# ShadowLive/ExtIO_sddc

Hardware: AMD Instinct MI355X
Metric: input MSamples/s at decim=2 + achieved % HBM roofline, 1 GPU; IQ max-rel-err (higher is better)
Workload: dtype f32 (int16 in, complex64 out)

## Files before the change

### extio_sddc_amd/csrc/ddc_fs.hip

```cpp
#include <hip/hip_runtime.h>

#include <type_traits>

#include "ddc_frame_common.hpp"
#include "ddc_queue.hpp"
#include "ddc_stamps.hpp"
#include "ddc_fs_perm.h"

namespace sddc {
namespace {

#ifdef SDDC_STAMPS
__device__ unsigned g_fs_stamps[2048 * 4 * kStampWords];
#endif

__device__ __forceinline__ float dpp_partner(float v)
{
    return __int_as_float(__builtin_amdgcn_mov_dpp(__float_as_int(v), 0xB1, 0xF, 0xF, true));
}

__device__ __forceinline__ void split_v2(float2 &za, float2 &vb, float2 zb, float ra, float rb)
{
    asm("s_nop 1\n\t"
        "v_fmac_f32_dpp %2, %1, %7 quad_perm:[1,0,3,2] row_mask:0xf bank_mask:0xf\n\t"
// ... 43 lines not shown
}

constexpr int kQWave = 3;
constexpr int kFsPqAhead = 1;
__device__ __forceinline__ int fs_row_slot(int t) { return 272 * (t >> 4) + (t >= 128) + 34 * ((t & 15) >> 1) + (t & 1); }
__device__ __forceinline__ int fs_pair_row(int t) { return 2 * (t >> 5) + (t & 1); }
__device__ __forceinline__ int fs_pair_col(int t) { return (t >> 1) & 15; }
__device__ __forceinline__ int fs_pair_slot(int t) { return t + 2 * (t >> 5); }
constexpr int kFsLds = 4352;
constexpr int kFsTw = NT + 1;

enum { kSchedStatic = 0, kSchedQueue = 1, kSchedSteal = 2 };
template <int SCHED> struct SchedOf { using T = StealSchedule; };
template <> struct SchedOf<kSchedStatic> { using T = StaticSchedule; };
template <> struct SchedOf<kSchedQueue> { using T = FrameSchedule<1>; };

template <int ZR>
__device__ __forceinline__ constexpr bool zrow(int k) { return zr_row<ZR>(k); }

template <int SCHED, int ZR, bool RAND, bool LSB, bool NCO, bool CS16>
__global__ __launch_bounds__(NT, 4) void r2iq_fs_kernel(
    const int *__restrict__ in32, void *__restrict__ out, int nframes, const float2 *__restrict__ tw_p1,
    const float2 *__restrict__ rec_f, const float4 *__restrict__ pqf, const float2 *__restrict__ fsl, int tunebin,
    OutArgs oa, NcoArgs nco, unsigned *__restrict__ wq, int ns, unsigned slotw, int xmap, int minrem, int pub)
{
    __shared__ __attribute__((aligned(16))) float2 lds[kFsLds];
    __shared__ __attribute__((aligned(16))) float2 twl[15 * 16];
    __shared__ __attribute__((aligned(16))) float2 wtab[2 * kFsTw];
    __shared__ int s_next;
    static_assert(sizeof(float2) * (kFsLds + 15 * 16 + 2 * kFsTw) + sizeof(int) <= 163840 / 4,
                  "four workgroups per CU");

    const int tid = (int)threadIdx.x;
    const int w = xmap ? (int)(blockIdx.x & 7u) * (int)(gridDim.x >> 3) + (int)(blockIdx.x >> 3) : (int)blockIdx.x;
    constexpr int QLANE = 64 * kQWave;
    const bool qw = __builtin_amdgcn_readfirstlane(tid >> 6) == kQWave;
    typename SchedOf<SCHED>::T fsch;
    int x[16];
    {
        const int G = (int)gridDim.x, a0 = slot_split(ns, G, w, slotw);
        const int f0s = a0 < slot_split(ns, G, w + 1, slotw) ? a0 : -1;
        if (f0s >= 0) load_frame(in32, f0s / FRAMES, f0s % FRAMES, x);
        if (qw) {
            int f0[1];
            if constexpr (SCHED == kSchedSteal) fsch.init(wq, nframes, ns, w, G, slotw, f0, minrem, pub);
            else fsch.init(wq, nframes, ns, w, G, slotw, f0);
            if (tid == QLANE) s_next = f0[0];
        }
        for (int i = tid; i < 15 * 16; i += NT) twl[i] = tw_p1[i];
        wtab[tid + (tid >= 128)] = rec_f[tid];
        wtab[kFsTw + tid + (tid >= 128)] = rec_f[NT + tid];
        __syncthreads();
        const int f = s_next;
        if (f >= 0 && f0s < 0) load_frame(in32, f / FRAMES, f % FRAMES, x);
    }
    int f = s_next;
    int blk = f / FRAMES, k = f - blk * FRAMES;
    const int col_ = kFsPerm[tid];
    const int qt = (tunebin >> 2) & 3;
    const bool w0 = __builtin_amdgcn_readfirstlane(tid >> 6) == 0;
    float cr[16];
    {
        const __amdgpu_buffer_rsrc_t rr = buf_rsrc(reinterpret_cast<const float *>(pqf) + 2 * HALF);
#pragma unroll
        for (int k = 0; k < 16; k++)
            if (!zrow<ZR>(k)) cr[k] = __uint_as_float(__builtin_amdgcn_raw_buffer_load_b32(rr, 4u * tid, 4u * NT * k, 0));
    }
    constexpr int AZR = ZR > 0 ? ZR : -ZR;
    constexpr int CPP = SCHED == kSchedStatic && !NCO && !CS16 && AZR >= 3 ? (AZR >= 4 && AZR <= 7 ? AZR + 1 : AZR) : 0;
    float2 cp[16];
    if constexpr (CPP > 0) {
        const __amdgpu_buffer_rsrc_t rq = buf_rsrc(pqf);
#pragma unroll
        for (int k = 0; k < 16; k++)
            if (!zrow<ZR>(k) && (k < CPP || 15 - k < CPP))
                cp[k] = buf_load8(rq, 16u * tid, 4096u * (k < 8 ? k : 15 - k) + (k < 8 ? 0u : 8u));
    }
    constexpr bool GREG = SCHED == kSchedStatic;
    float2 cg0, cg1, cg4;
    if constexpr (GREG) {
        const __amdgpu_buffer_rsrc_t rfs = buf_rsrc(fsl);
        const unsigned t8 = 8u * (unsigned)tid;
        cg0 = buf_load8(rfs, t8, 0);
        cg1 = buf_load8(rfs, t8, 8u * NT);
        cg4 = buf_load8(rfs, t8, 16u * NT);
    }
    int pA = -1, fend = -1;
    {
        const int G = (int)gridDim.x, a = slot_split(ns, G, w, slotw), b = slot_split(ns, G, w + 1, slotw);
        if constexpr (SCHED == kSchedStatic) {
            pA = b + 2;
            fend = b;
        } else if constexpr (SCHED == kSchedSteal) {
            const int len = b - a, two = len < 2 ? len : 2;
            pA = minrem <= 0 ? b + 2 : a + (pub > 0 && len - pub > two ? len - pub : two);
            fend = minrem <= 0 ? b : pA;
        }
    }
    ST_INIT();

    auto frame = [&](auto phase) __attribute__((always_inline)) {
        constexpr bool PB = decltype(phase)::value;
        if constexpr (PB && SCHED != kSchedSteal)
            if (qw) fsch.peek();
        int z = 0;
        asm volatile("" : "+s"(z));
        const int t = tid + z;
        const int c = col_ + z;
        const int oblk = blk * 8 * HALF;
        const int kc = k;
        float2 v[16];
        {
// ... 191 lines not shown
            const int fb = oblk + emit_base<HALF>(kc);
            switch (qt) {
            case 0: emit_frame_q<0, LSB, NCO, CS16>(out, fb, kc, t, u, oa, nco); break;
            case 1: emit_frame_q<1, LSB, NCO, CS16>(out, fb, kc, t, u, oa, nco); break;
            case 2: emit_frame_q<2, LSB, NCO, CS16>(out, fb, kc, t, u, oa, nco); break;
            default: emit_frame_q<3, LSB, NCO, CS16>(out, fb, kc, t, u, oa, nco); break;
            }
        }
        if constexpr (SCHED == kSchedSteal) {
            if constexpr (PB)
                if (qw) fsch.take_late();
        }
        ST_FRAME_END();
        f = fn;
    };
    if constexpr (SCHED != kSchedQueue)
        while (f >= 0 && f + 2 < pA) frame(std::false_type{});
    if constexpr (SCHED != kSchedStatic) {
        if constexpr (SCHED == kSchedSteal)
            if (qw) fsch.enter(f);
        while (f >= 0) frame(std::true_type{});
    }
    ST_WRITE(g_fs_stamps, w, tid);
    if constexpr (SCHED == kSchedQueue)
        if (tid == QLANE) fs_queue_done(wq, (unsigned)gridDim.x);
}

__global__ void build_fs_tables_kernel(const float2 *__restrict__ hsel0, const float2 *__restrict__ post8192,
                                       const float2 *__restrict__ tw4096, int tunebin, float4 *__restrict__ pqf,
                                       float2 *__restrict__ fsl)
{
    const int i = (int)(blockIdx.x * blockDim.x + threadIdx.x);
    if (i >= HALF) return;
    const int l = i & (NT - 1), kk = i >> 8;
    const int b = kFsPerm[l] + NT * kk;
    const bool band = (b >= tunebin && b - tunebin < HALF / 2) || (b < tunebin && tunebin - b <= HALF / 2);
    float3 c = make_float3(0.f, 0.f, 0.f);
    if (band) {
        const int m = (b - tunebin) & (HALF - 1);
        const double hr = hsel0[m].x, hi = hsel0[m].y;
        const double wr = post8192[b].x, wi = post8192[b].y;
        const double pr = 1.0 + wi, pi = -wr, qr = 1.0 - wi, qi = wr;
        if (b == HALF / 2) {
            c.x = (float)(hr * qr - hi * qi);
            c.y = (float)(hr * qi + hi * qr);
        } else {
// ... 6 lines not shown
    reinterpret_cast<float *>(pqf)[2 * HALF + i] = c.z;
    if (i < NT) {
        fsl[i] = tw4096[(tunebin * i) & (HALF - 1)];
        fsl[NT + i] = tw4096[((tunebin - 1) * i) & (HALF - 1)];
        fsl[2 * NT + i] = tw4096[((tunebin - 4) * i) & (HALF - 1)];
    }
}

template <int SCHED, int ZR, bool RAND, bool LSB, bool NCO, bool CS16>
hipError_t launch_fs_s(const KernelTables &t, const int16_t *d_in, int nblk, void *d_out, const float4 *pqf,
                       const float2 *fsl, int tunebin, const OutArgs &oa, const NcoArgs &nco, unsigned *wq,
                       const FsSched &fs, int device, hipStream_t s)
{
    auto kern = r2iq_fs_kernel<SCHED, ZR, RAND, LSB, NCO, CS16>;
    const int static_pct = SCHED == kSchedQueue ? fs.static_pct : 100, fpw = fs.fpw;
    int occ = 0, cus = 0;
    hipError_t e = launch_geometry(t.lc, reinterpret_cast<const void *>(kern), NT, device, &occ, &cus);
    if (e != hipSuccess) return e;
    const int nframes = nblk * FRAMES;
    int grid = cus * occ;
    if (grid > nframes) grid = nframes;
    int ns = frame_schedule_static(nframes, static_pct);
    unsigned slotw = occ == 4 && grid == cus * occ ? (fs.slotw ? fs.slotw : kFsSlotWeights) : 0u;
    int xmap = 0;
    if (fpw > 0) {
        grid = (nframes + fpw - 1) / fpw;
        ns = nframes;
        slotw = 0u;
        xmap = (grid & 7) == 0 && grid * fpw == nframes;
    }
    int minrem = fs.minrem;
    if (SCHED == kSchedSteal && (grid > kFsStealMax || 2LL * nframes / grid + 1 > kStealMaxRange)) minrem = 0;
    hipLaunchKernelGGL(kern, dim3((unsigned)grid), dim3(NT), 0, s, reinterpret_cast<const int *>(d_in), d_out, nframes,
                       t.tw_p1, t.rec_f, pqf, fsl, tunebin, oa, nco, wq, ns, slotw, xmap, minrem, fs.pub);
    return hipGetLastError();
}

int fs_zero_rows(int tunebin)
{
    const int top = 16 - (tunebin + 2048 + 255) / 256, bot = tunebin > 2048 ? (tunebin - 2048) / 256 : 0;
    const int z = top > 0 ? top : bot > 0 ? -bot : 0;
    return z > 8 ? 8 : z < -8 ? -8 : z == 1 || z == -1 ? 0 : z;
}

template <int ZR, bool RAND, bool LSB, bool NCO, bool CS16>
hipError_t launch_fs_z(const KernelTables &t, const int16_t *d_in, int nblk, void *d_out, const float4 *pqf,
                       const float2 *fsl, int tunebin, const OutArgs &oa, const NcoArgs &nco, unsigned *wq,
                       const FsSched &fs, int device, hipStream_t s)
{
    if (fs.sched == kSchedStatic)
        return launch_fs_s<kSchedStatic, ZR, RAND, LSB, NCO, CS16>(t, d_in, nblk, d_out, pqf, fsl, tunebin, oa, nco, wq, fs, device, s);
    if constexpr (!RAND && !LSB && !NCO && !CS16 && ZR % 4 == 0) {
        if (fs.sched == kSchedSteal)
            return launch_fs_s<kSchedSteal, ZR, false, false, false, false>(t, d_in, nblk, d_out, pqf, fsl, tunebin, oa, nco, wq, fs, device, s);
        if (fs.sched == kSchedQueue)
            return launch_fs_s<kSchedQueue, ZR, false, false, false, false>(t, d_in, nblk, d_out, pqf, fsl, tunebin, oa, nco, wq, fs, device, s);
    }
// ... 80 lines not shown
```

### extio_sddc_amd/csrc/ddc_kernels.h

```cpp
#pragma once

#include <hip/hip_runtime_api.h>
#include <hip/hip_vector_types.h>
#include <stddef.h>
#include <stdint.h>

namespace sddc {

struct LaunchCache {
    static constexpr int kSlots = 256;
    int cus = 0;
    int n = 0;
    const void *fn[kSlots] = {};
    int occ[kSlots] = {};
};

inline hipError_t launch_geometry(LaunchCache *lc, const void *fn, int threads, int device, int *occ, int *cus)
{
    if (lc) {
        for (int i = 0; i < lc->n; i++)
            if (lc->fn[i] == fn) {
                *occ = lc->occ[i];
                *cus = lc->cus;
                return hipSuccess;
            }
    }
    int nb = 0, c = 0;
    hipError_t e = hipOccupancyMaxActiveBlocksPerMultiprocessor(&nb, fn, threads, 0);
// ... 28 lines not shown
                                    const float2 *nco_trig, int slot_weights, int device, hipStream_t s);
constexpr unsigned slot_weights4(unsigned a, unsigned b, unsigned c, unsigned e) { return a | (b << 8) | (c << 16) | (e << 24); }
constexpr unsigned kSlotWeights[7] = {slot_weights4(31, 26, 18, 13), slot_weights4(31, 26, 18, 13), slot_weights4(31, 26, 18, 13),
                                      slot_weights4(29, 25, 20, 15), slot_weights4(29, 25, 20, 15),
                                      slot_weights4(29, 25, 20, 15), slot_weights4(29, 25, 20, 15)};
constexpr int kSlotWeighting = 1;
hipError_t launch_build_split_filter(const KernelTables &t, int d, int tunebin, float4 *pq, hipStream_t s);

bool fs_path(int d, int tunebin);
hipError_t launch_build_fs_tables(const KernelTables &t, int tunebin, float4 *pqf, float2 *fsl, hipStream_t s);
constexpr int kFsQueueLineWords = 16 * 9;
constexpr int kFsStealMax = 2048;
constexpr int kFsQueueWords = kFsQueueLineWords + 2 * kFsStealMax;
constexpr int kFsStaticPct = 100;
constexpr unsigned kFsSlotWeights = slot_weights4(31, 26, 18, 13);
struct FsSched {
    int sched = 0;
    int static_pct = kFsStaticPct;
    int fpw = 0;
    int minrem = 1;
    int pub = 0;
    int zr = 1;
    unsigned slotw = 0u;
};
hipError_t launch_frames_fs(const KernelTables &t, const int16_t *d_in, int nblk, void *d_out, const float4 *pqf,
                            const float2 *fsl, int tunebin, int lsb, int rand, int cs16, float cs16_scale,
                            const float2 *nco_starts, const float2 *nco_trig, unsigned *wq, const FsSched &fs,
                            int device, hipStream_t s);

struct ChNco {
    const float2 *starts = nullptr;
    const float2 *trig = nullptr;
    const float *fc = nullptr;
    int nb = 0;
};
hipError_t launch_channel_nco_chain(float2 *d_state, const float2 *d_trig, float2 *d_starts, int nch, int nb,
                                    hipStream_t s);

hipError_t launch_channels_v2(const KernelTables &t, int d, const int16_t *d_in, int nblk, const int *d_tunebins,
                              int nch, void *d_out, size_t stride, int lsb, int rand, int cs16, float cs16_scale,
                              const int2 *d_windows, float2 *d_scratch, int scratch_rows, int device,
                              hipStream_t s, const ChNco *nco = nullptr);
hipError_t launch_channels_p(const KernelTables &t, int d, const int16_t *d_in, int nblk, const int *d_tunebins,
                             int nch, void *d_out, size_t stride, int lsb, int rand, int cs16, float cs16_scale,
                             float2 *d_scratch, int scratch_rows, int device, hipStream_t s,
                             const ChNco *nco = nullptr);
// ... 8 lines not shown
```

### extio_sddc_amd/csrc/ddc_queue.hpp

```cpp
#pragma once

#include <hip/hip_runtime.h>

#include "ddc_device_io.hpp"

namespace sddc {
namespace {

constexpr int FS_SHARDS = 8;
static_assert(kFsQueueLineWords == 16 * (FS_SHARDS + 1), "queue slot: one 64-B line per shard counter + the done count");
constexpr unsigned FS_OOB = 0x80000000u;

__device__ __forceinline__ int slot_split(int ns, int G, int v, unsigned slotw)
{
    if (slotw == 0u || (G & 3)) return (int)(((long long)ns * v) / G);
    const int Q = G >> 2, q = v / Q, i = v - q * Q;
    long long sw = 0, tot = 0;
#pragma unroll
    for (int k = 0; k < 4; k++) {
        const int wk = (int)((slotw >> (8 * k)) & 0xffu);
        tot += (long long)Q * wk;
        if (k < q) sw += (long long)Q * wk;
        else if (k == q) sw += (long long)i * wk;
    }
    return (int)(((long long)ns * sw) / tot);
}

struct FsQueue {
    __amdgpu_buffer_rsrc_t rq;
    int base, nd;
    int sh0;
    int shn;
    int lo, cnt;
    int tk;
    int pv;

    __device__ __forceinline__ int shard_lo(int s) const { return base + ((nd * s) >> 3); }
    __device__ __forceinline__ void init(unsigned *wq, int base_, int nd_, int home)
    {
        rq = __builtin_amdgcn_make_buffer_rsrc(wq, (short)0, 4 * kFsQueueLineWords, 0x00020000);
        base = base_;
        nd = nd_;
        sh0 = home;
        set_shard(0);
    }
    __device__ __forceinline__ void set_shard(int sh)
    {
        shn = sh;
// ... 51 lines not shown
        }
        rem = b - a - LA;
        nxt = a + LA;
        if (rem <= 0) q.take();
    }
    __device__ __forceinline__ void peek()
    {
        if (rem <= 0) q.peek();
    }
    __device__ __forceinline__ int next()
    {
        const int fn = rem > 0 ? nxt++ : q.resolve();
        rem--;
        return fn;
    }
    __device__ __forceinline__ void take()
    {
        if (rem <= 0) q.take();
    }
};

struct StaticSchedule {
    int nxt, end;
    __device__ __forceinline__ void init(unsigned *, int, int ns, int w, int G, unsigned slotw, int (&f)[1])
    {
        const int a = slot_split(ns, G, w, slotw), b = slot_split(ns, G, w + 1, slotw);
        f[0] = a < b ? a : -1;
        nxt = a + 1;
        end = b;
    }
    __device__ __forceinline__ void peek() {}
    __device__ __forceinline__ int next() { return nxt < end ? nxt++ : -1; }
    __device__ __forceinline__ void take() {}
};

constexpr unsigned kStealBias = 0x4000u;
constexpr int kStealMaxRange = 0x3fff;
static_assert(kFsQueueWords >= kFsQueueLineWords + 2 * kFsStealMax, "queue slot: queue lines + steal slots");
constexpr unsigned STEAL_OOB = 0x80000000u;

__device__ __forceinline__ int steal_front(unsigned x) { return (int)(x >> 16); }
__device__ __forceinline__ int steal_end(unsigned x) { return (int)(x & 0xffffu) - (int)kStealBias; }

struct StealSchedule {
    enum { kOwn, kScan, kSteal, kDone, kPriv, kStatic };
    __amdgpu_buffer_rsrc_t rs;
// ... 147 lines not shown
```

### extio_sddc_amd/csrc/ddc_runtime.cpp

```cpp
#include <hip/hip_runtime_api.h>

#include <algorithm>
#include <cmath>
#include <complex>
#include <cstdarg>
#include <cstdio>
#include <cstdlib>
#include <cstring>
#include <memory>
#include <mutex>
#include <new>
#include <string>
#include <vector>

#include "cpu/r2iq_cpu.h"
#include "ddc_kernels.h"
#include "filterbank.h"
#include "fine_tune.h"
#include "sddc_fft.h"
#include "sddc_ddc.h"
#include "sddc_ddc_internal.h"

namespace {

thread_local std::string g_last_error;

int fail(int code, const char *fmt, ...)
{
    char buf[512];
    va_list ap;
    va_start(ap, fmt);
    vsnprintf(buf, sizeof buf, fmt, ap);
    va_end(ap);
    g_last_error = buf;
    return code;
}

#define HIP_TRY(expr)                                                                         \
    do {                                                                                      \
        hipError_t e_ = (expr);                                                               \
        if (e_ != hipSuccess)                                                                 \
// ... 101 lines not shown
    int last_slot = -1, last_n = 0;
    std::vector<std::pair<const char *, size_t>> regions;

    int *d_tunebins = nullptr;
    std::vector<int> tunebins_cached;
    int2 *d_windows = nullptr;
    int windows_d = -1;
    float2 *d_chscratch = nullptr;
    int chscratch_rows = 0;
    Readers ch_readers;

    float4 *d_pq = nullptr;
    int pq_d = -1, pq_tb = -1;
    hipStream_t pq_s = nullptr;
    float4 *d_fs = nullptr;
    int fs_tb = -1;
    hipStream_t fs_s = nullptr;
    static constexpr int kQueueSlots = 64;
    unsigned *d_queue = nullptr;
    int queue_slot = 0;
    int slot_weights = sddc::kSlotWeighting;
    sddc::FsSched fs_sched;
    hipStream_t q_s[kQueueSlots] = {};
    bool q_used[kQueueSlots] = {};
    bool q_dirty[kQueueSlots] = {};
    Readers readers;

    float nco_fc = 0.f;
    sddc::FineTune nco;
    static constexpr int kNcoSlots = 3;
    float2 *h_nco[kNcoSlots] = {};
    hipEvent_t nco_ev[kNcoSlots] = {};
    size_t h_nco_cap = 0;
    int nco_slot = 0;
    float2 *d_nco = nullptr;
    size_t d_nco_cap = 0;

    std::vector<float> chnco_fc;
    float2 *d_chnco_trig = nullptr;
    float2 *d_chnco_state = nullptr;
    float *d_chnco_fc = nullptr;
    float2 *d_chnco_starts = nullptr;
    size_t chnco_starts_cap = 0;
    int chnco_run_blocks = 0;

    std::vector<int16_t> hist_override;
// ... 197 lines not shown
        (void)h->ch_readers.sync();
        if (h->d_tables) (void)hipFree(h->d_tables);
        for (auto &sl : h->hs) {
            if (sl.d_in) (void)hipFree(sl.d_in);
            if (sl.d_out) (void)hipFree(sl.d_out);
            if (sl.h_in) (void)hipHostFree(sl.h_in);
            if (sl.h_out) (void)hipHostFree(sl.h_out);
            for (hipEvent_t ev : {sl.e_h2d, sl.e_k, sl.e_d2h})
                if (ev) (void)hipEventDestroy(ev);
        }
        if (h->s_in) (void)hipStreamDestroy(h->s_in);
        if (h->s_out) (void)hipStreamDestroy(h->s_out);
        for (auto &r : h->regions) (void)hipHostUnregister(const_cast<char *>(r.first));
        if (h->d_tunebins) (void)hipFree(h->d_tunebins);
        if (h->d_windows) (void)hipFree(h->d_windows);
        if (h->d_chscratch) (void)hipFree(h->d_chscratch);
        if (h->d_chnco_trig) (void)hipFree(h->d_chnco_trig);
        if (h->d_chnco_state) (void)hipFree(h->d_chnco_state);
        if (h->d_chnco_fc) (void)hipFree(h->d_chnco_fc);
        if (h->d_chnco_starts) (void)hipFree(h->d_chnco_starts);
        if (h->d_pq) (void)hipFree(h->d_pq);
        if (h->d_fs) (void)hipFree(h->d_fs);
        if (h->d_queue) (void)hipFree(h->d_queue);
        h->readers.clear();
        h->ch_readers.clear();
        for (int i = 0; i < sddc_ddc::kNcoSlots; i++) {
            if (h->h_nco[i]) (void)hipHostFree(h->h_nco[i]);
            if (h->nco_ev[i]) (void)hipEventDestroy(h->nco_ev[i]);
        }
        if (h->d_nco) (void)hipFree(h->d_nco);
        if (h->stream) (void)hipStreamDestroy(h->stream);
    }
    delete h;
    return SDDC_OK;
}

int sddc_ddc_set_decimation(sddc_ddc_t *h, int d)
{
    if (!h) return fail(SDDC_ERR_ARG, "null handle");
    if (d < 0 || d >= SDDC_DDC_NDEC) return fail(SDDC_ERR_ARG, "decimation index %d outside 0..6", d);
    std::lock_guard<std::mutex> lk(h->mu);
    h->d = d;
    return SDDC_OK;
}

int sddc_ddc_set_sideband(sddc_ddc_t *h, int lsb)
// ... 134 lines not shown
    return e;
}

static void queue_slot_launched(sddc_ddc_t *h, int i, hipStream_t s, hipError_t e)
{
    h->q_s[i] = s;
    h->q_used[i] = true;
    if (e != hipSuccess) {
        h->q_dirty[i] = true;
        (void)h->readers.record(s);
    }
}

static void queue_mark_all_dirty(sddc_ddc_t *h)
{
    for (int i = 0; i < sddc_ddc::kQueueSlots; i++) h->q_dirty[i] = true;
}

static hipError_t order_after_build(sddc_ddc_t *h, hipStream_t built, hipStream_t s)
{
    return h->readers.order_after(built, s);
}

static hipError_t launch_single_impl(sddc_ddc_t *h, const int16_t *d_in, int nblk, void *d_out, hipStream_t s);

static hipError_t launch_single(sddc_ddc_t *h, const int16_t *d_in, int nblk, void *d_out, hipStream_t s)
{
    const hipError_t e = launch_single_impl(h, d_in, nblk, d_out, s);
    if (e != hipSuccess) queue_mark_all_dirty(h);
    return e;
}

static hipError_t launch_single_impl(sddc_ddc_t *h, const int16_t *d_in, int nblk, void *d_out, hipStream_t s)
{
    const bool nco = h->nco_fc != 0.f;
    if (nco) {
        hipError_t e = stage_nco(h, nblk, s);
        if (e != hipSuccess) return e;
    }
    const float2 *nco_starts = nco ? h->d_nco + sddc::FineTune::kTable : nullptr, *nco_trig = nco ? h->d_nco : nullptr;
    if (sddc::fs_path(h->d, h->tunebin)) {
        float4 *pqf = h->d_fs;
        float2 *fsl = reinterpret_cast<float2 *>(h->d_fs + 4096);
        if (h->fs_tb != h->tunebin) {
            hipError_t e = h->readers.order_before(s);
            if (e != hipSuccess) return e;
            h->fs_tb = -1;
            e = sddc::launch_build_fs_tables(h->tables, h->tunebin, pqf, fsl, s);
            if (e == hipSuccess) e = h->readers.record(s);
            if (e != hipSuccess) return e;
            h->fs_tb = h->tunebin;
            h->fs_s = s;
        } else if (hipError_t e = order_after_build(h, h->fs_s, s); e != hipSuccess) {
            return e;
        }
        unsigned *wq = nullptr;
        int qi = -1;
        hipError_t e = hipSuccess;
        if (h->fs_sched.sched != 0 && (e = next_queue_slot(h, s, &wq, &qi)) != hipSuccess) return e;
        e = sddc::launch_frames_fs(h->tables, d_in, nblk, d_out, pqf, fsl, h->tunebin, h->lsb, h->rand,
                                   h->out_fmt == SDDC_DDC_FMT_CS16, h->cs16_scale, nco_starts, nco_trig, wq,
                                   h->fs_sched, h->device, s);
        if (qi >= 0) queue_slot_launched(h, qi, s, e);
        if (e != hipSuccess) return e;
        return h->readers.record(s);
    }
    if (h->pq_d != h->d || h->pq_tb != h->tunebin) {
        hipError_t e = h->readers.order_before(s);
        if (e != hipSuccess) return e;
        h->pq_d = h->pq_tb = -1;
        e = sddc::launch_build_split_filter(h->tables, h->d, h->tunebin, h->d_pq, s);
        if (e == hipSuccess) e = h->readers.record(s);
        if (e != hipSuccess) return e;
        h->pq_d = h->d;
        h->pq_tb = h->tunebin;
        h->pq_s = s;
    } else if (hipError_t e = order_after_build(h, h->pq_s, s); e != hipSuccess) {
        return e;
    }
    hipError_t e = sddc::launch_frames_persistent(h->tables, h->d, d_in, nblk, d_out, h->d_pq, h->tunebin, h->lsb, h->rand,
                                         h->out_fmt == SDDC_DDC_FMT_CS16, h->cs16_scale, nco_starts, nco_trig,
                                         h->slot_weights, h->device, s);
// ... 100 lines not shown
    case SDDC_DDC_PARAM_FS_SCHEDULE:
        if (value < 0 || value > 2) return fail(SDDC_ERR_ARG, "FS schedule %d outside 0..2", value);
        h->fs_sched.sched = value;
        return SDDC_OK;
    case SDDC_DDC_PARAM_FS_STEAL_MINREM:
        if (value < 0 || value > 64) return fail(SDDC_ERR_ARG, "steal threshold %d outside 0..64", value);
        h->fs_sched.minrem = value;
        return SDDC_OK;
    case SDDC_DDC_PARAM_FS_ZERO_ROWS:
        h->fs_sched.zr = value != 0;
        return SDDC_OK;
    case SDDC_DDC_PARAM_FS_SLOT_WEIGHTS: {
        for (int k = 0; k < 4 && value != 0; k++) {
            const int wk = (value >> (8 * k)) & 0xff;
            if (wk < 1 || wk > 127) return fail(SDDC_ERR_ARG, "slot weight %d of slot %d outside 1..127", wk, k);
        }
        h->fs_sched.slotw = (unsigned)value;
        return SDDC_OK;
    }
    case SDDC_DDC_PARAM_FS_STEAL_PUBLIC:
        if (value < 0 || value > 1024) return fail(SDDC_ERR_ARG, "public frames %d outside 0..1024", value);
        h->fs_sched.pub = value;
        return SDDC_OK;
    case SDDC_DDC_PARAM_CH_NCO_RUN_BLOCKS:
        if (value < 0 || value > SDDC_DDC_MAX_BLOCKS)
            return fail(SDDC_ERR_ARG, "run blocks %d outside 0..%d", value, SDDC_DDC_MAX_BLOCKS);
        h->chnco_run_blocks = value;
        return SDDC_OK;
    default:
        return fail(SDDC_ERR_ARG, "unknown parameter %d", param);
    }
}

static int check_process_args(sddc_ddc_t *h, const int16_t *in, int nblk, const void *out)
{
    if (!h) return fail(SDDC_ERR_ARG, "null handle");
    if (nblk <= 0 || nblk > SDDC_DDC_MAX_BLOCKS)
        return fail(SDDC_ERR_ARG, "nblk must be in 1..%d (got %d)", SDDC_DDC_MAX_BLOCKS, nblk);
    if (!in || !out) return fail(SDDC_ERR_ARG, "null buffer");
    if (((uintptr_t)in & 3) != 0) return fail(SDDC_ERR_ARG, "input must be 4-byte aligned");
    const unsigned oal = h->out_fmt == SDDC_DDC_FMT_CS16 ? 4 : 8;
    if (((uintptr_t)out & (oal - 1)) != 0) return fail(SDDC_ERR_ARG, "output must be %u-byte aligned", oal);
    return SDDC_OK;
}

int sddc_ddc_process_device(sddc_ddc_t *h, const int16_t *d_in, int nblk, void *d_out, void *hip_stream)
{
    if (!h) return fail(SDDC_ERR_ARG, "null handle");
    std::lock_guard<std::mutex> lk(h->mu);
    if (h->cpu) return fail(SDDC_ERR_STATE, "process_device: a CPU handle has no device path");
    int rc = check_process_args(h, d_in, nblk, d_out);
    if (rc) return rc;
    if (injected_failure(h)) return fail(SDDC_ERR_HIP, "injected failure (SDDC_DDC_INJECT_FAIL)");
    DeviceGuard g(h->device);
// ... 347 lines not shown
```

### extio_sddc_amd/csrc/sddc_ddc_internal.h

```cpp
#pragma once
#include "sddc_ddc.h"
#ifdef __cplusplus
extern "C" {
#endif
#define SDDC_DDC_PARAM_FS_STATIC_PCT 1
#define SDDC_DDC_PARAM_SLOT_WEIGHTS 2
#define SDDC_DDC_PARAM_FS_FRAMES_PER_WG 3
#define SDDC_DDC_PARAM_FS_SCHEDULE 4
#define SDDC_DDC_PARAM_FS_STEAL_MINREM 5
#define SDDC_DDC_PARAM_FS_STEAL_PUBLIC 6
#define SDDC_DDC_PARAM_FS_ZERO_ROWS 7
#define SDDC_DDC_PARAM_FS_SLOT_WEIGHTS 8
#define SDDC_DDC_PARAM_CH_NCO_RUN_BLOCKS 9

int sddc_ddc_internal_set_param(sddc_ddc_t *h, int param, int value);
int sddc_ddc_internal_fs_stamps(unsigned *host, int nwords, int *words_per_wave);
int sddc_ddc_internal_p_stamps(unsigned *host, int nwords, int *words_per_wave);
#ifdef __cplusplus
}
#endif
```

Baseline: 649,000.

## Add adaptive per-workgroup frame split driven by measured kernel timings

Under the static schedule, each workgroup can now log its start and end realtime stamps into a host-mapped ring buffer. A host-side controller learns a per-workgroup cost and start-offset model from these stamps and computes a quantized share table, so later launches assign more frames to faster slots and fewer to slower ones. The goal is to reduce tail imbalance between workgroups that the fixed slot weights leave behind. In exchange it adds host bookkeeping per launch, a mapped-memory write per workgroup, a larger kernel argument, and frame assignments that depend on runtime measurements and can adapt poorly.

New measurement: 662,700, median of 6. 1.02x the previous value.

```diff
diff --git a/extio_sddc_amd/csrc/ddc_fs.hip b/extio_sddc_amd/csrc/ddc_fs.hip
--- a/extio_sddc_amd/csrc/ddc_fs.hip
+++ b/extio_sddc_amd/csrc/ddc_fs.hip
@@ -89,7 +89,8 @@
 __global__ __launch_bounds__(NT, 4) void r2iq_fs_kernel(
     const int *__restrict__ in32, void *__restrict__ out, int nframes, const float2 *__restrict__ tw_p1,
     const float2 *__restrict__ rec_f, const float4 *__restrict__ pqf, const float2 *__restrict__ fsl, int tunebin,
-    OutArgs oa, NcoArgs nco, unsigned *__restrict__ wq, int ns, unsigned slotw, int xmap, int minrem, int pub)
+    OutArgs oa, NcoArgs nco, unsigned *__restrict__ wq, int ns, unsigned slotw, int xmap, int minrem, int pub,
+    unsigned *__restrict__ tlog, unsigned ttag, int use_tab, FsShares shares)
 {
     __shared__ __attribute__((aligned(16))) float2 lds[kFsLds];
     __shared__ __attribute__((aligned(16))) float2 twl[15 * 16];
@@ -103,14 +104,22 @@
     constexpr int QLANE = 64 * kQWave;
     const bool qw = __builtin_amdgcn_readfirstlane(tid >> 6) == kQWave;
     typename SchedOf<SCHED>::T fsch;
+    auto split = [&](int G, int v) __attribute__((always_inline)) {
+        if constexpr (SCHED == kSchedStatic) return fs_static_split(ns, G, v, slotw, use_tab, shares);
+        else return slot_split(ns, G, v, slotw);
+    };
+    unsigned t_start = 0u;
+    if constexpr (SCHED == kSchedStatic)
+        if (tlog) t_start = (unsigned)__builtin_amdgcn_s_memrealtime();
     int x[16];
     {
-        const int G = (int)gridDim.x, a0 = slot_split(ns, G, w, slotw);
-        const int f0s = a0 < slot_split(ns, G, w + 1, slotw) ? a0 : -1;
+        const int G = (int)gridDim.x, a0 = split(G, w), b0 = split(G, w + 1);
+        const int f0s = a0 < b0 ? a0 : -1;
         if (f0s >= 0) load_frame(in32, f0s / FRAMES, f0s % FRAMES, x);
         if (qw) {
             int f0[1];
             if constexpr (SCHED == kSchedSteal) fsch.init(wq, nframes, ns, w, G, slotw, f0, minrem, pub);
+            else if constexpr (SCHED == kSchedStatic) fsch.init_range(a0, b0, f0);
             else fsch.init(wq, nframes, ns, w, G, slotw, f0);
             if (tid == QLANE) s_next = f0[0];
         }
@@ -154,7 +163,7 @@
     }
     int pA = -1, fend = -1;
     {
-        const int G = (int)gridDim.x, a = slot_split(ns, G, w, slotw), b = slot_split(ns, G, w + 1, slotw);
+        const int G = (int)gridDim.x, a = split(G, w), b = split(G, w + 1);
         if constexpr (SCHED == kSchedStatic) {
             pA = b + 2;
             fend = b;
@@ -392,6 +401,12 @@
         while (f >= 0) frame(std::true_type{});
     }
     ST_WRITE(g_fs_stamps, w, tid);
+    if constexpr (SCHED == kSchedStatic) {
+        if (tlog && tid == 0) {
+            const unsigned t_end = (unsigned)__builtin_amdgcn_s_memrealtime();
+            reinterpret_cast<uint4 *>(tlog)[w] = make_uint4(t_start, t_end, ttag, t_start ^ t_end ^ ttag);
+        }
+    }
     if constexpr (SCHED == kSchedQueue)
         if (tid == QLANE) fs_queue_done(wq, (unsigned)gridDim.x);
 }
@@ -444,6 +459,14 @@
     if (grid > nframes) grid = nframes;
     int ns = frame_schedule_static(nframes, static_pct);
     unsigned slotw = occ == 4 && grid == cus * occ ? (fs.slotw ? fs.slotw : kFsSlotWeights) : 0u;
+    const FsShares *tab = nullptr;
+    unsigned *tlog = nullptr, ttag = 0u;
+    if (SCHED == kSchedStatic && fs.adapt && slotw != 0u && fs.slotw == 0u && fpw <= 0 && grid <= kFsShareMaxG &&
+        !fs.adapt(fs.adapt_ctx, grid, ns, &tab, &tlog, &ttag)) {
+        tab = nullptr;
+        tlog = nullptr;
+    }
+    static const FsShares kNoShares = {};
     int xmap = 0;
     if (fpw > 0) {
         grid = (nframes + fpw - 1) / fpw;
@@ -454,7 +477,8 @@
     int minrem = fs.minrem;
     if (SCHED == kSchedSteal && (grid > kFsStealMax || 2LL * nframes / grid + 1 > kStealMaxRange)) minrem = 0;
     hipLaunchKernelGGL(kern, dim3((unsigned)grid), dim3(NT), 0, s, reinterpret_cast<const int *>(d_in), d_out, nframes,
-                       t.tw_p1, t.rec_f, pqf, fsl, tunebin, oa, nco, wq, ns, slotw, xmap, minrem, fs.pub);
+                       t.tw_p1, t.rec_f, pqf, fsl, tunebin, oa, nco, wq, ns, slotw, xmap, minrem, fs.pub, tlog, ttag,
+                       tab ? 1 : 0, tab ? *tab : kNoShares);
     return hipGetLastError();
 }
 
diff --git a/extio_sddc_amd/csrc/ddc_kernels.h b/extio_sddc_amd/csrc/ddc_kernels.h
--- a/extio_sddc_amd/csrc/ddc_kernels.h
+++ b/extio_sddc_amd/csrc/ddc_kernels.h
@@ -4,6 +4,8 @@
 #include <hip/hip_vector_types.h>
 #include <stddef.h>
 #include <stdint.h>
+
+#include "fs_shares.h"
 
 namespace sddc {
 
@@ -78,6 +80,8 @@
     int pub = 0;
     int zr = 1;
     unsigned slotw = 0u;
+    bool (*adapt)(void *ctx, int G, int ns, const FsShares **tab, unsigned **tlog, unsigned *tag) = nullptr;
+    void *adapt_ctx = nullptr;
 };
 hipError_t launch_frames_fs(const KernelTables &t, const int16_t *d_in, int nblk, void *d_out, const float4 *pqf,
                             const float2 *fsl, int tunebin, int lsb, int rand, int cs16, float cs16_scale,
diff --git a/extio_sddc_amd/csrc/ddc_queue.hpp b/extio_sddc_amd/csrc/ddc_queue.hpp
--- a/extio_sddc_amd/csrc/ddc_queue.hpp
+++ b/extio_sddc_amd/csrc/ddc_queue.hpp
@@ -24,6 +24,11 @@
         else if (k == q) sw += (long long)i * wk;
     }
     return (int)(((long long)ns * sw) / tot);
+}
+
+__device__ __forceinline__ int fs_static_split(int ns, int G, int v, unsigned slotw, int tab, const FsShares &sh)
+{
+    return tab ? fs_share_start(ns, G, v, sh) : slot_split(ns, G, v, slotw);
 }
 
 struct FsQueue {
@@ -121,6 +126,12 @@
 
 struct StaticSchedule {
     int nxt, end;
+    __device__ __forceinline__ void init_range(int a, int b, int (&f)[1])
+    {
+        f[0] = a < b ? a : -1;
+        nxt = a + 1;
+        end = b;
+    }
     __device__ __forceinline__ void init(unsigned *, int, int ns, int w, int G, unsigned slotw, int (&f)[1])
     {
         const int a = slot_split(ns, G, w, slotw), b = slot_split(ns, G, w + 1, slotw);
diff --git a/extio_sddc_amd/csrc/ddc_runtime.cpp b/extio_sddc_amd/csrc/ddc_runtime.cpp
--- a/extio_sddc_amd/csrc/ddc_runtime.cpp
+++ b/extio_sddc_amd/csrc/ddc_runtime.cpp
@@ -17,6 +17,7 @@
 #include "ddc_kernels.h"
 #include "filterbank.h"
 #include "fine_tune.h"
+#include "fs_split_controller.hpp"
 #include "sddc_fft.h"
 #include "sddc_ddc.h"
 #include "sddc_ddc_internal.h"
@@ -164,6 +165,34 @@
     int slot_weights = sddc::kSlotWeighting;
     sddc::FsSched fs_sched;
     hipStream_t q_s[kQueueSlots] = {};
+
+    struct FsAdapt {
+        static constexpr int kRing = 16;
+        static constexpr int kTaint = 4;
+        static constexpr int kEager = 32;
+        static constexpr int kEvery = 8;
+        bool on = true;
+        sddc::FsSplitController ctl;
+        std::vector<float> forced;
+        unsigned *h_ring = nullptr, *d_ring = nullptr;
+        bool ring_failed = false;
+        struct Pending {
+            unsigned tag = 0u;
+            int G = 0, ns = 0;
+            bool live = false, tainted = false;
+            std::vector<int> n;
+        } pend[kRing];
+        int next = 0, last_pending = -1;
+        unsigned seq = 0u;
+        sddc::FsShares tab = {};
+        std::vector<int> tab_n, base_n;
+        int tab_ns = -1, base_ns = -1;
+        hipStream_t cur_s = nullptr, last_s = nullptr;
+        bool have_last = false;
+        int taint_left = 0;
+        long launches = 0, skipped = 0;
+        int last_table = 0, last_logged = 0;
+    } fsa;
     bool q_used[kQueueSlots] = {};
     bool q_dirty[kQueueSlots] = {};
     Readers readers;
@@ -407,6 +436,7 @@
         if (h->d_pq) (void)hipFree(h->d_pq);
         if (h->d_fs) (void)hipFree(h->d_fs);
         if (h->d_queue) (void)hipFree(h->d_queue);
+        if (h->fsa.h_ring) (void)hipHostFree(h->fsa.h_ring);
         h->readers.clear();
         h->ch_readers.clear();
         for (int i = 0; i < sddc_ddc::kNcoSlots; i++) {
@@ -587,6 +617,103 @@
     return h->readers.order_after(built, s);
 }
 
+static bool fs_adapt_prepare(void *ctx, int G, int ns, const sddc::FsShares **tab, unsigned **tlog, unsigned *tag)
+{
+    using sddc::kFsShareMaxG;
+    sddc_ddc_t *h = static_cast<sddc_ddc_t *>(ctx);
+    sddc_ddc::FsAdapt &a = h->fsa;
+    const bool want_forced = (int)a.forced.size() == G;
+    if (!a.on && !want_forced) return false;
+    if (a.ctl.groups() != G) a.ctl.reset(G, sddc::kFsSlotWeights);
+    if (want_forced && !a.ctl.forced()) a.ctl.load(a.forced.data(), G);
+    if (!want_forced && a.ctl.forced()) a.ctl.unload();
+    a.ctl.set_frames(ns);
+    const bool learn = a.on && !a.ctl.forced();
+    bool changed = false;
+    if (learn && a.h_ring) {
+        const bool take = a.ctl.measured() < sddc_ddc::FsAdapt::kEager || a.launches % sddc_ddc::FsAdapt::kEvery == 0;
+        for (int k = 0; k < sddc_ddc::FsAdapt::kRing && take; k++) {
+            auto &p = a.pend[(a.next + k) % sddc_ddc::FsAdapt::kRing];
+            if (!p.live) continue;
+            const volatile unsigned *e = a.h_ring + (size_t)((a.next + k) % sddc_ddc::FsAdapt::kRing) * kFsShareMaxG * 4;
+            bool done = true;
+            for (int w = 0; w < p.G && done; w++)
+                done = e[4 * w + 2] == p.tag && (e[4 * w] ^ e[4 * w + 1] ^ p.tag) == e[4 * w + 3];
+            if (!done) continue;
+            p.live = false;
+            if (p.tainted || p.G != G || p.ns != ns) {
+                a.skipped++;
+                continue;
+            }
+            uint32_t st[kFsShareMaxG], en[kFsShareMaxG];
+            for (int w = 0; w < G; w++) {
+                st[w] = e[4 * w];
+                en[w] = e[4 * w + 1];
+            }
+            if (a.ctl.update(p.n.data(), st, en)) changed = true;
+            else a.skipped++;
+        }
+    }
+    a.launches++;
+    const std::vector<int> *n = nullptr;
+    if (a.ctl.warm()) {
+        if (changed || a.tab_ns != ns) {
+            a.tab_n.resize((size_t)G);
+            a.ctl.table(ns, &a.tab, a.tab_n.data());
+            a.tab_ns = ns;
+        }
+        *tab = &a.tab;
+        n = &a.tab_n;
+        a.last_table = 1;
+    } else {
+        if (a.base_ns != ns || (int)a.base_n.size() != G) {
+            a.base_n.resize((size_t)G);
+            for (int w = 0; w < G; w++)
+                a.base_n[(size_t)w] = sddc::fs_slot_split_host(ns, G, w + 1, sddc::kFsSlotWeights) -
+                                      sddc::fs_slot_split_host(ns, G, w, sddc::kFsSlotWeights);
+            a.base_ns = ns;
+        }
+        *tab = nullptr;
+        n = &a.base_n;
+    }
+    *tlog = nullptr;
+    *tag = 0u;
+    if (!learn) return true;
+    if (!a.h_ring && !a.ring_failed) {
+        const size_t bytes = (size_t)sddc_ddc::FsAdapt::kRing * kFsShareMaxG * 4 * sizeof(unsigned);
+        void *hp = nullptr, *dp = nullptr;
+        if (hipHostMalloc(&hp, bytes, hipHostMallocMapped) == hipSuccess) {
+            if (hipHostGetDevicePointer(&dp, hp, 0) == hipSuccess) {
+                std::memset(hp, 0, bytes);
+                a.h_ring = static_cast<unsigned *>(hp);
+                a.d_ring = static_cast<unsigned *>(dp);
+            } else {
+                (void)hipHostFree(hp);
+            }
+        }
+        if (!a.h_ring) {
+            a.ring_failed = true;
+            (void)hipGetLastError();
+        }
+    }
+    if (!a.h_ring) return true;
+    const int i = a.next;
+    a.next = (i + 1) % sddc_ddc::FsAdapt::kRing;
+    if (++a.seq == 0u) a.seq = 1u;
+    auto &p = a.pend[i];
+    p.tag = a.seq;
+    p.G = G;
+    p.ns = ns;
+    p.live = true;
+    p.tainted = a.taint_left > 0;
+    p.n = *n;
+    a.last_pending = i;
+    a.last_logged = 1;
+    *tlog = a.d_ring + (size_t)i * kFsShareMaxG * 4;
+    *tag = p.tag;
+    return true;
+}
+
 static hipError_t launch_single_impl(sddc_ddc_t *h, const int16_t *d_in, int nblk, void *d_out, hipStream_t s);
 
 static hipError_t launch_single(sddc_ddc_t *h, const int16_t *d_in, int nblk, void *d_out, hipStream_t s)
@@ -598,6 +725,19 @@
 
 static hipError_t launch_single_impl(sddc_ddc_t *h, const int16_t *d_in, int nblk, void *d_out, hipStream_t s)
 {
+    {
+        sddc_ddc::FsAdapt &a = h->fsa;
+        if (a.have_last && a.last_s != s) {
+            a.taint_left = sddc_ddc::FsAdapt::kTaint + 1;
+            if (a.last_pending >= 0) a.pend[a.last_pending].tainted = true;
+        } else if (a.taint_left > 0) {
+            a.taint_left--;
+        }
+        a.last_s = s;
+        a.have_last = true;
+        a.last_pending = -1;
+        a.last_table = a.last_logged = 0;
+    }
     const bool nco = h->nco_fc != 0.f;
     if (nco) {
         hipError_t e = stage_nco(h, nblk, s);
@@ -623,6 +763,8 @@
         int qi = -1;
         hipError_t e = hipSuccess;
         if (h->fs_sched.sched != 0 && (e = next_queue_slot(h, s, &wq, &qi)) != hipSuccess) return e;
+        h->fs_sched.adapt = fs_adapt_prepare;
+        h->fs_sched.adapt_ctx = h;
         e = sddc::launch_frames_fs(h->tables, d_in, nblk, d_out, pqf, fsl, h->tunebin, h->lsb, h->rand,
                                    h->out_fmt == SDDC_DDC_FMT_CS16, h->cs16_scale, nco_starts, nco_trig, wq,
                                    h->fs_sched, h->device, s);
@@ -769,6 +911,9 @@
         if (value < 0 || value > 1024) return fail(SDDC_ERR_ARG, "public frames %d outside 0..1024", value);
         h->fs_sched.pub = value;
         return SDDC_OK;
+    case SDDC_DDC_PARAM_FS_ADAPTIVE_SPLIT:
+        h->fsa.on = value != 0;
+        return SDDC_OK;
     case SDDC_DDC_PARAM_CH_NCO_RUN_BLOCKS:
         if (value < 0 || value > SDDC_DDC_MAX_BLOCKS)
             return fail(SDDC_ERR_ARG, "run blocks %d outside 0..%d", value, SDDC_DDC_MAX_BLOCKS);
@@ -777,6 +922,89 @@
     default:
         return fail(SDDC_ERR_ARG, "unknown parameter %d", param);
     }
+}
+
+int sddc_ddc_internal_fs_set_shares(sddc_ddc_t *h, const float *shares, int n)
+{
+    if (!h) return fail(SDDC_ERR_ARG, "null handle");
+    if (n < 0 || n > sddc::kFsShareMaxG || (n > 0 && !shares)) return fail(SDDC_ERR_ARG, "shares: n %d outside 0..%d", n, sddc::kFsShareMaxG);
+    double sum = 0.0;
+    for (int w = 0; w < n; w++) {
+        if (!(shares[w] >= 0.f) || !std::isfinite(shares[w])) return fail(SDDC_ERR_ARG, "share %d is negative or not finite", w);
+        sum += shares[w];
+    }
+    if (n > 0 && !(sum > 0.0)) return fail(SDDC_ERR_ARG, "shares: all zero");
+    std::lock_guard<std::mutex> lk(h->mu);
+    h->fsa.forced.assign(shares, shares + n);
+    if (h->fsa.ctl.forced()) h->fsa.ctl.unload();
+    h->fsa.tab_ns = -1;
+    return SDDC_OK;
+}
+
+int sddc_ddc_internal_fs_split_state(sddc_ddc_t *h, long *info, int *counts, int ncounts)
+{
+    if (!h) return fail(SDDC_ERR_ARG, "null handle");
+    std::lock_guard<std::mutex> lk(h->mu);
+    const sddc_ddc::FsAdapt &a = h->fsa;
+    if (info) {
+        info[0] = a.ctl.groups();
+        info[1] = a.ctl.measured();
+        info[2] = a.skipped;
+        info[3] = a.last_table;
+        info[4] = a.last_logged;
+    }
+    int nw = 0;
+    if (counts && a.tab_ns >= 0 && ncounts >= (int)a.tab_n.size()) {
+        nw = (int)a.tab_n.size();
+        std::copy(a.tab_n.begin(), a.tab_n.end(), counts);
+    }
+    return nw;
+}
+
+void *sddc_fs_split_create(int G, unsigned slot_weights)
+{
+    if (G < 1 || G > sddc::kFsShareMaxG) return nullptr;
+    auto *c = new (std::nothrow) sddc::FsSplitController;
+    if (c) c->reset(G, slot_weights);
+    return c;
+}
+void sddc_fs_split_destroy(void *c) { delete static_cast<sddc::FsSplitController *>(c); }
+int sddc_fs_split_load(void *c, const float *shares, int n)
+{
+    auto *k = static_cast<sddc::FsSplitController *>(c);
+    if (n == 0) {
+        k->unload();
+        return 0;
+    }
+    return k->load(shares, n) ? 0 : -1;
+}
+int sddc_fs_split_table(void *c, int ns, unsigned *p, int *first)
+{
+    auto *k = static_cast<sddc::FsSplitController *>(c);
+    const int G = k->groups();
+    if (ns < 0) return -1;
+    sddc::FsShares t;
+    std::vector<int> n((size_t)G);
+    k->table(ns, &t, n.data());
+    if (!sddc::fs_shares_valid(t, G)) return -2;
+    for (int w = 0; w <= G; w++) {
+        if (p) p[w] = w < G ? sddc::fs_share_get(t, w) : sddc::kFsShareOne;
+        if (first) first[w] = sddc::fs_share_start(ns, G, w, t);
+    }
+    return 0;
+}
+int sddc_fs_split_update(void *c, const int *n, const unsigned *start, const unsigned *end)
+{
+    return static_cast<sddc::FsSplitController *>(c)->update(n, start, end) ? 1 : 0;
+}
+int sddc_fs_split_model(void *c, double *cost, double *offset)
+{
+    auto *k = static_cast<sddc::FsSplitController *>(c);
+    for (int w = 0; w < k->groups(); w++) {
+        if (cost) cost[w] = k->cost()[(size_t)w];
+        if (offset) offset[w] = k->offset()[(size_t)w];
+    }
+    return k->groups();
 }
 
 static int check_process_args(sddc_ddc_t *h, const int16_t *in, int nblk, const void *out)
diff --git a/extio_sddc_amd/csrc/fs_shares.h b/extio_sddc_amd/csrc/fs_shares.h
--- /dev/null
+++ b/extio_sddc_amd/csrc/fs_shares.h
@@ -0,0 +1,53 @@
+#pragma once
+
+#include <stdint.h>
+
+#if defined(__HIPCC__)
+#define SDDC_HD __host__ __device__
+#else
+#define SDDC_HD
+#endif
+
+namespace sddc {
+
+constexpr int kFsShareMaxG = 1024;
+constexpr int kFsShareBits = 15;
+constexpr unsigned kFsShareOne = 1u << kFsShareBits;
+
+struct FsShares {
+    uint32_t p[kFsShareMaxG / 2];
+};
+
+SDDC_HD inline unsigned fs_share_get(const FsShares &t, int v) { return (t.p[v >> 1] >> (16 * (v & 1))) & 0xffffu; }
+inline void fs_share_set(FsShares &t, int v, unsigned pv)
+{
+    const int sh = 16 * (v & 1);
+    t.p[v >> 1] = (t.p[v >> 1] & ~(0xffffu << sh)) | ((pv & 0xffffu) << sh);
+}
+
+SDDC_HD inline int fs_share_start(int ns, int G, int v, const FsShares &t)
+{
+    if (v >= G) return ns;
+    return (int)(((long long)ns * (long long)fs_share_get(t, v)) >> kFsShareBits);
+}
+
+inline unsigned fs_share_of(long long A, int ns)
+{
+    if (ns <= 0 || A <= 0) return 0u;
+    if (A >= ns) return kFsShareOne;
+    return (unsigned)((A * (long long)kFsShareOne + ns - 1) / ns);
+}
+
+inline bool fs_shares_valid(const FsShares &t, int G)
+{
+    if (G < 1 || G > kFsShareMaxG) return false;
+    unsigned last = 0u;
+    for (int v = 0; v < G; v++) {
+        const unsigned pv = fs_share_get(t, v);
+        if (pv < last || pv > kFsShareOne) return false;
+        last = pv;
+    }
+    return true;
+}
+
+}
diff --git a/extio_sddc_amd/csrc/fs_split_controller.hpp b/extio_sddc_amd/csrc/fs_split_controller.hpp
--- /dev/null
+++ b/extio_sddc_amd/csrc/fs_split_controller.hpp
@@ -0,0 +1,213 @@
+#pragma once
+
+#include <stdint.h>
+
+#include <algorithm>
+#include <cmath>
+#include <vector>
+
+#include "fs_shares.h"
+
+namespace sddc {
+
+inline int fs_slot_split_host(int ns, int G, int v, unsigned slotw)
+{
+    if (slotw == 0u || (G & 3)) return (int)(((long long)ns * v) / G);
+    const int Q = G >> 2, q = v / Q, i = v - q * Q;
+    long long sw = 0, tot = 0;
+    for (int k = 0; k < 4; k++) {
+        const int wk = (int)((slotw >> (8 * k)) & 0xffu);
+        tot += (long long)Q * wk;
+        if (k < q) sw += (long long)Q * wk;
+        else if (k == q) sw += (long long)i * wk;
+    }
+    return (int)(((long long)ns * sw) / tot);
+}
+
+class FsSplitController {
+public:
+    static constexpr double kEta = 0.25;
+    static constexpr double kStep = 1.25;
+    static constexpr double kClamp = 0.25;
+    static constexpr double kCostSpan = 2.0;
+    static constexpr double kMaxOffset = 8.0;
+
+    void reset(int G, unsigned slotw)
+    {
+        G_ = G;
+        slotw_ = slotw;
+        measured_ = 0;
+        ns_ = 0;
+        c0_.assign((size_t)G, 1.0);
+        if (slotw != 0u && !(G & 3)) {
+            double sum = 0.0;
+            for (int k = 0; k < 4; k++) sum += (double)((slotw >> (8 * k)) & 0xffu);
+            for (int w = 0; w < G; w++) c0_[(size_t)w] = sum / 4.0 / (double)((slotw >> (8 * (w / (G >> 2)))) & 0xffu);
+        }
+        c_ = c0_;
+        o_.assign((size_t)G, 0.0);
+        forced_.clear();
+    }
+    int groups() const { return G_; }
+    unsigned slot_weights() const { return slotw_; }
+    long measured() const { return measured_; }
+    bool forced() const { return !forced_.empty(); }
+    bool warm() const { return forced() || measured_ > 0; }
+    const std::vector<double> &cost() const { return c_; }
+    const std::vector<double> &offset() const { return o_; }
+
+    void set_frames(int ns)
+    {
+        if (ns != ns_ && measured_ > 0) {
+            const std::vector<double> f = forced_;
+            reset(G_, slotw_);
+            forced_ = f;
+        }
+        ns_ = ns;
+    }
+
+    bool load(const float *shares, int n)
+    {
+        if (n != G_ || !shares) return false;
+        double sum = 0.0;
+        for (int w = 0; w < n; w++) {
+            if (!(shares[w] >= 0.f) || !std::isfinite(shares[w])) return false;
+            sum += shares[w];
+        }
+        if (!(sum > 0.0)) return false;
+        forced_.resize((size_t)n);
+        for (int w = 0; w < n; w++) forced_[(size_t)w] = shares[w] / sum;
+        return true;
+    }
+    void unload() { forced_.clear(); }
+
+    void allocate(int ns, int *n) const
+    {
+        const int G = G_;
+        if (forced()) {
+            double cum = 0.0;
+            long long prev = 0;
+            for (int w = 0; w < G; w++) {
+                cum += forced_[(size_t)w];
+                long long A = w == G - 1 ? ns : (long long)std::floor(cum * ns + 0.5);
+                A = std::min<long long>(std::max(A, prev), ns);
+                n[w] = (int)(A - prev);
+                prev = A;
+            }
+            return;
+        }
+        lo_.resize((size_t)G);
+        hi_.resize((size_t)G);
+        ic_.resize((size_t)G);
+        double tmax = 0.0;
+        for (int w = 0; w < G; w++) {
+            const int base = fs_slot_split_host(ns, G, w + 1, slotw_) - fs_slot_split_host(ns, G, w, slotw_);
+            lo_[(size_t)w] = (int)(base * (1.0 - kClamp));
+            hi_[(size_t)w] = (int)std::ceil(base * (1.0 + kClamp));
+            ic_[(size_t)w] = 1.0 / c_[(size_t)w];
+            tmax = std::max(tmax, o_[(size_t)w] + (hi_[(size_t)w] + 1) * c_[(size_t)w]);
+        }
+        auto count = [&](double T, int *out) {
+            long long tot = 0;
+            for (int w = 0; w < G; w++) {
+                const double x = (T - o_[(size_t)w]) * ic_[(size_t)w];
+                int k = x > 0.0 ? (x < 2.0e9 ? (int)x : 2000000000) : 0;
+                k = std::min(std::max(k, lo_[(size_t)w]), hi_[(size_t)w]);
+                if (out) out[w] = k;
+                tot += k;
+            }
+            return tot;
+        };
+        double a = 0.0, b = tmax;
+        for (int it = 0; it < 40; it++) {
+            const double T = 0.5 * (a + b);
+            if (count(T, nullptr) >= ns) b = T;
+            else a = T;
+        }
+        long long extra = count(b, n) - ns;
+        while (extra > 0) {
+            int best = -1;
+            double be = -1.0;
+            for (int w = 0; w < G; w++) {
+                const double e = o_[(size_t)w] + n[w] * c_[(size_t)w];
+                if (n[w] > lo_[(size_t)w] && e > be) be = e, best = w;
+            }
+            if (best < 0) break;
+            n[best]--;
+            extra--;
+        }
+        while (extra < 0) {
+            int best = -1;
+            double be = 1e300;
+            for (int w = 0; w < G; w++) {
+                const double e = o_[(size_t)w] + (n[w] + 1) * c_[(size_t)w];
+                if (n[w] < hi_[(size_t)w] && e < be) be = e, best = w;
+            }
+            if (best < 0) break;
+            n[best]++;
+            extra++;
+        }
+        if (extra != 0) n[G - 1] = (int)std::max<long long>(0, n[G - 1] - extra);
+    }
+
+    void table(int ns, FsShares *t, int *n) const
+    {
+        const int G = G_;
+        allocate(ns, n);
+        long long A = 0;
+        for (int w = 0; w < kFsShareMaxG / 2; w++) t->p[w] = 0u;
+        for (int w = 0; w < G; w++) {
+            fs_share_set(*t, w, fs_share_of(A, ns));
+            A += n[w];
+        }
+        for (int w = 0; w < G; w++) n[w] = fs_share_start(ns, G, w + 1, *t) - fs_share_start(ns, G, w, *t);
+    }
+
+    bool update(const int *n, const uint32_t *start, const uint32_t *end)
+    {
+        const int G = G_;
+        if (forced()) return false;
+        double sum_d = 0.0;
+        long long sum_n = 0;
+        int32_t first = 0;
+        for (int w = 0; w < G; w++) {
+            const uint32_t d = end[w] - start[w];
+            if (n[w] < 0 || d > 0x40000000u || (n[w] > 0 && d == 0u)) return false;
+            const int32_t rel = (int32_t)(start[w] - start[0]);
+            first = std::min(first, rel);
+            sum_d += n[w] > 0 ? (double)d : 0.0;
+            sum_n += n[w];
+        }
+        if (sum_n <= 0 || !(sum_d > 0.0)) return false;
+        const double m = sum_d / (double)sum_n;
+        double norm = 0.0;
+        for (int w = 0; w < G; w++) {
+            double &c = c_[(size_t)w];
+            if (n[w] > 0) {
+                const double obs = (double)(end[w] - start[w]) / (n[w] * m);
+                const double r = std::min(std::max(obs / c, 1.0 / kStep), kStep);
+                c *= 1.0 + kEta * (r - 1.0);
+            }
+            const double so = std::min((double)((int32_t)(start[w] - start[0]) - first) / m, kMaxOffset);
+            o_[(size_t)w] += kEta * (so - o_[(size_t)w]);
+            norm += c / c0_[(size_t)w];
+        }
+        norm /= G;
+        for (int w = 0; w < G; w++) {
+            const double c0 = c0_[(size_t)w];
+            c_[(size_t)w] = std::min(std::max(c_[(size_t)w] / norm, c0 / kCostSpan), c0 * kCostSpan);
+        }
+        measured_++;
+        return true;
+    }
+
+private:
+    int G_ = 0, ns_ = 0;
+    unsigned slotw_ = 0u;
+    long measured_ = 0;
+    std::vector<double> c0_, c_, o_, forced_;
+    mutable std::vector<int> lo_, hi_;
+    mutable std::vector<double> ic_;
+};
+
+}
diff --git a/extio_sddc_amd/csrc/sddc_ddc_internal.h b/extio_sddc_amd/csrc/sddc_ddc_internal.h
--- a/extio_sddc_amd/csrc/sddc_ddc_internal.h
+++ b/extio_sddc_amd/csrc/sddc_ddc_internal.h
@@ -12,8 +12,17 @@
 #define SDDC_DDC_PARAM_FS_ZERO_ROWS 7
 #define SDDC_DDC_PARAM_FS_SLOT_WEIGHTS 8
 #define SDDC_DDC_PARAM_CH_NCO_RUN_BLOCKS 9
+#define SDDC_DDC_PARAM_FS_ADAPTIVE_SPLIT 10
 
 int sddc_ddc_internal_set_param(sddc_ddc_t *h, int param, int value);
+int sddc_ddc_internal_fs_set_shares(sddc_ddc_t *h, const float *shares, int n);
+int sddc_ddc_internal_fs_split_state(sddc_ddc_t *h, long *info, int *counts, int ncounts);
+void *sddc_fs_split_create(int G, unsigned slot_weights);
+void sddc_fs_split_destroy(void *c);
+int sddc_fs_split_load(void *c, const float *shares, int n);
+int sddc_fs_split_table(void *c, int ns, unsigned *p, int *first);
+int sddc_fs_split_update(void *c, const int *n, const unsigned *start, const unsigned *end);
+int sddc_fs_split_model(void *c, double *cost, double *offset);
 int sddc_ddc_internal_fs_stamps(unsigned *host, int nwords, int *words_per_wave);
 int sddc_ddc_internal_p_stamps(unsigned *host, int nwords, int *words_per_wave);
 #ifdef __cplusplus
```
